# davawen/Simple-Raytracer

Measured on AMD Instinct MI355X. Metric: Mray/s at 1920x1080x1024spp, higher is better.
Workload: dtype f32; 1 GPU; BASELINE configs[1]: 7-shape sphere scene 1920x1080 1024spp; width=1920, height=1080, spp=1024, bounces=10, triangles=12, partition=single GPU, gather=none, mode=parity (fp-contract off, IEEE div/sqrt; canvas bit-identical to the CPU oracle)

## Files before the change

### simple-raytracer_amd/csrc/device_types.h

```cpp
#ifndef SRT_DEVICE_TYPES_H
#define SRT_DEVICE_TYPES_H

#include <stddef.h>
#include <stdint.h>

#include "../../include/srt_types.h"

struct ShapeRun {
	int32_t type;
	uint32_t first_shape;
	uint32_t count;
	uint32_t data_off;
};
struct BlockGroup {
	uint32_t code;
	uint32_t first[3];
};
static_assert(sizeof(BlockGroup) == 16, "BlockGroup 16 B");

struct WinnerRec {
	int32_t type;
	int32_t material;
	float vx, vy, vz, w;
	uint32_t first_wtri;
	float inv_w;
};
static_assert(sizeof(WinnerRec) == 32, "WinnerRec 32 B");

#define SRT_WTRI_FLOATS 9

typedef srt_bvh_node BvhNode;
#define SRT_BVH_FIRST_DWORD 11
#define SRT_BVH_TRI_FLOATS 9
#define SRT_BVH_LEAF_J 28
#define SRT_BVH_NONE 0xffffffffu
#define SRT_BVH_LEAF_BIT 0x80000000u
#define SRT_BVH_INDEX_MASK 0x0fffffffu
#define SRT_BVH_INDEX_MAX 0x01ffffffu
#define SRT_BVH_KEY_INF 0x7f800000u
#define SRT_BVH_TAG_MASK 31u
#define SRT_BVH_TAG_LEAF 16u
#define SRT_BVH_TAG(ref, slot) ((((ref) >> 31) << 4) | ((((ref) >> 28) & 3u) << 2) | (slot))
#define SRT_BVH_STACK_CAP 64
#ifndef SRT_BVH_LEAF_MAX
#define SRT_BVH_LEAF_MAX 3
#endif

#define SRT_REGION_MAX 56
#ifdef SRT_REGION_COUNT
#define SRT_WAVE_CTR_STRIDE (16 + 2 * SRT_REGION_MAX)
#else
#define SRT_WAVE_CTR_STRIDE 16
#endif
#define SRT_WAVE_CTR_SLOTS 8192

enum { SRT_CTR_RAYS = 0, SRT_CTR_SKY, SRT_CTR_TRI, SRT_CTR_TRI_PASS_U, SRT_CTR_NAN, SRT_CTR_PATHS, SRT_CTR_QUEUE, SRT_CTR_WATCHDOG, SRT_CTR_QUEUE2, SRT_CTR_COUNT };

#define SRT_MF_NO_SPECULAR 1
#define SRT_MF_PLAIN_COLORS 2

#define SRT_BLK_CODE(type, count) ((uint32_t)((type) + 1) | ((uint32_t)(count) << 2))
#define SRT_GROUP_CODE(b0, b1, b2) ((b0) | ((b1) << 8) | ((b2) << 16))
#define SRT_GC_PPS SRT_GROUP_CODE(SRT_BLK_CODE(SRT_SHAPE_PLANE, 2), SRT_BLK_CODE(SRT_SHAPE_PLANE, 1), SRT_BLK_CODE(SRT_SHAPE_SPHERE, 4))
#define SRT_GC_SSS SRT_GROUP_CODE(SRT_BLK_CODE(SRT_SHAPE_SPHERE, 4), SRT_BLK_CODE(SRT_SHAPE_SPHERE, 4), SRT_BLK_CODE(SRT_SHAPE_SPHERE, 4))
#define SRT_GC_PPP SRT_GROUP_CODE(SRT_BLK_CODE(SRT_SHAPE_PLANE, 2), SRT_BLK_CODE(SRT_SHAPE_PLANE, 2), SRT_BLK_CODE(SRT_SHAPE_PLANE, 2))
#define SRT_SCENE_CLASS_LIST(X) \
	X(1, SRT_GC_PPS, true)      \
	X(2, SRT_GC_PPS, false)     \
	X(3, SRT_GC_SSS, true)      \
	X(4, SRT_GC_PPP, true)
#define SRT_SCENE_CLASS_GENERAL 0

static inline size_t srt_scene_lds_bytes(size_t num_shapes, size_t num_materials, int num_models, size_t num_runs) {
	size_t scene = num_shapes * sizeof(WinnerRec) + num_materials * sizeof(srt_material);
	if (num_models == 0) scene += num_runs * (sizeof(BlockGroup) + 192);
	return scene <= 4608 ? scene : 0;
}

struct TraceParams {
	srt_render_data rd;
	srt_scene_data sd;
	const BlockGroup *runs;
	const float *run_data;
	const WinnerRec *winners;
	int32_t num_runs;
	int32_t num_materials;
	uint32_t lds_bytes;
	int32_t scene_class;
	const srt_shape *shapes;
	const srt_triangle *triangles;
	const srt_material *materials;
	const float *wtris;
	const float *sky;
	float *canvas;
	float *radiance;
	unsigned long long *counters;
	unsigned long long *wave_counters;
	unsigned long long *queue;
	unsigned long long total_items;
	uint32_t batch_samples;
	uint32_t first_sample;
	uint32_t job_items;
	uint32_t stage_off;
	int32_t sky_w, sky_h;
	float f_width, f_height, f_sky_w, f_sky_h;
	int32_t sun_focus_int;
	int32_t material_flags;
	int32_t num_models;
	int32_t rank, world, rows_per_block, owned_rows;
	int32_t use_bvh;
	const float *bvh_blocks;
	float *scan_queue;
	float inv_f_width, inv_f_height;
	uint32_t width_magic, width_shift;
	uint32_t rpb_magic, rpb_shift;
	uint32_t nbs_magic16;
	uint32_t pool_blocks;
	int32_t unit_materials;
	int32_t all_materials_ok;
};

static inline void srt_magic_u31(uint32_t d, uint32_t *magic, uint32_t *shift) {
	uint32_t l = 0;
	while (l < 32 && ((uint64_t)1 << l) < d) l++;
// ... 125 lines not shown
```

### simple-raytracer_amd/csrc/kernels.hip

```cpp
#include <hip/hip_runtime.h>

#include "detmath.h"
#include "device_types.h"
#include "tonemap.h"

#ifndef SRT_TEXTURED
#define SRT_TEXTURED 0
#endif
#if SRT_TEXTURED
#define SRT_TRACE_PARAMS TexTraceParams
#define SRT_FEATURE_PARAMS TexFeatureParams
#define srt_trace_kernel srt_trace_tex_kernel
#define srt_features_kernel srt_features_tex_kernel
#define srt_features_ids_kernel srt_features_ids_tex_kernel
#define srt_launch_trace srt_launch_trace_tex
#define srt_trace_resident_waves_per_cu srt_trace_tex_resident_waves_per_cu
#define srt_launch_features srt_launch_features_tex
#define srt_launch_features_ids srt_launch_features_ids_tex
int srt_trace_lds_floats(int has_models, int use_bvh);
#else
#define SRT_TRACE_PARAMS TraceParams
#define SRT_FEATURE_PARAMS FeatureParams
#endif

// ... 311 lines not shown
		tmin = t_key;
		best = idx;
	}
}

template <int N>
__device__ __forceinline__ void test_spheres(const Blk16 &s, f3 org, f3 dir, int idx0, float &tmin, int &best) {
	float bq[4], disc[4];
	bool slow = is_neg_zero(tmin);
#pragma unroll
	for (int i = 0; i < N; i++) {
		f3 L = mk(s.v[4 * i] - org.x, s.v[4 * i + 1] - org.y, s.v[4 * i + 2] - org.z);
		bq[i] = dot3(L, dir);
		float c = dot3(L, L) - s.v[4 * i + 3];
		disc[i] = bq[i] * bq[i] - c;
		slow = slow || dm_fabs(disc[i]) < 0x1p-96f;
	}
	if (__builtin_expect(any64(slow), 0)) {
#pragma unroll
		for (int i = 0; i < N; i++) {
			const float sq = __builtin_sqrtf(disc[i]);
			float t = bq[i] - sq;
			if (t < 0.0f) t = bq[i] + sq;
			if (!(disc[i] < 0.0f) && !(t < 0.0f) && t < tmin) tmin = t, best = idx0 + i;
		}
	} else {
		float dd[N], sq[N];
#pragma unroll
		for (int i = 0; i < N; i++) dd[i] = disc[i];
		sqrt_rsq_n<N, false>(dd, sq);
#pragma unroll
		for (int i = 0; i < N; i++) {
			const uint32_t k = min(dm_f2u(bq[i] - sq[i]), dm_f2u(bq[i] + sq[i]));
			take_if_closer(dm_u2f(k), idx0 + i, tmin, best);
		}
	}
}

__device__ __forceinline__ void test_planes2(const Blk16 &b, uint32_t count, f3 org, f3 dir, int idx0, float &tmin, int &best) {
#pragma unroll
	for (int i = 0; i < 2; i++) {
		if (i == 1 && count < 2u) break;
		f3 n = mk(b.v[8 * i + 4], b.v[8 * i + 5], b.v[8 * i + 6]);
		float denom = dot3(n, dir);
		float t = dot3(n, mk(b.v[8 * i] - org.x, b.v[8 * i + 1] - org.y, b.v[8 * i + 2] - org.z)) / denom;
		bool hit = !(t < 0.0f);
		if (hit && t < tmin) {
			tmin = t;
			best = idx0 + i;
		}
	}
}

__device__ __forceinline__ bool test_aabb(float lx, float ly, float lz, float hx, float hy, float hz, f3 org, f3 inv, float tmax) {
	float t0 = 0.0f, t1 = tmax;
	float a1 = (lx - org.x) * inv.x, a2 = (hx - org.x) * inv.x;
	t0 = dm_max(t0, dm_min(a1, a2));
	t1 = dm_min(t1, dm_max(a1, a2));
	a1 = (ly - org.y) * inv.y, a2 = (hy - org.y) * inv.y;
	t0 = dm_max(t0, dm_min(a1, a2));
	t1 = dm_min(t1, dm_max(a1, a2));
	a1 = (lz - org.z) * inv.z, a2 = (hz - org.z) * inv.z;
	t0 = dm_max(t0, dm_min(a1, a2));
	t1 = dm_min(t1, dm_max(a1, a2));
	return t0 < t1;
}

template <bool COUNT_TRIS>
__device__ __forceinline__ bool moller_trumbore(float v0x, float v0y, float v0z, float e1x, float e1y, float e1z, float e2x, float e2y,
                                                float e2z, f3 org, f3 dir, bool counted, float &t, uint32_t &n_tri_u SRT_RC_PARAM) {
	f3 e1 = mk(e1x, e1y, e1z), e2 = mk(e2x, e2y, e2z);
	f3 h = cross3(dir, e2);
	float a = dot3(e1, h);
	f3 sv = mk(org.x - v0x, org.y - v0y, org.z - v0z);
	float sh = dot3(sv, h);
	float aa = dm_fabs(a), ash = dm_fabs(sh);
	bool reject = (a == 0.0f) || (ash > aa * 1.001f) || ((sh * a < 0.0f) && (ash >= aa * 0.001f));
	bool ok = false;
	if (!reject) {
		SRT_REGION(EXTEND_TRI_EXACT);
		f3 q = cross3(sv, e1);
		float dv = dot3(dir, q);
		bool reject2 = false;
		if (!COUNT_TRIS) reject2 = ((dv * a < 0.0f) && (dm_fabs(dv) >= aa * 0.001f)) || (dm_fabs(sh + dv) > aa * 1.01f);
		if (!reject2) {
			SRT_REGION(EXTEND_TRI_DIV);
			float f = 1.0f / a;
			float u = f * sh;
			ok = !(u < 0.0f || u > 1.0f);
			if (COUNT_TRIS) n_tri_u += (ok && counted) ? 1u : 0u;
			float v = f * dv;
			ok = ok && !(v < 0.0f || u + v > 1.0f);
			t = f * dot3(e2, q);
			ok = ok && t > 0.0f;
		}
	}
	return ok;
}

template <bool COUNT_TRIS>
__device__ __forceinline__ void test_triangle(float v0x, float v0y, float v0z, float e1x, float e1y, float e1z, float e2x, float e2y,
                                              float e2z, f3 org, f3 dir, int idx, uint32_t j, uint32_t count, float &tmin, int &best,
                                              uint32_t &best_tri, uint32_t &n_tri_u SRT_RC_PARAM) {
	float t = 0.0f;
	if (moller_trumbore<COUNT_TRIS>(v0x, v0y, v0z, e1x, e1y, e1z, e2x, e2y, e2z, org, dir, j < count, t, n_tri_u SRT_RC_ARG) && t < tmin) {
		tmin = t;
// ... 371 lines not shown
__device__ __forceinline__ uint32_t popc64(unsigned long long m) { return (uint32_t)__builtin_popcountll(m); }
__device__ __forceinline__ uint32_t lane_rank(unsigned long long m) {
	return __builtin_amdgcn_mbcnt_hi((uint32_t)(m >> 32), __builtin_amdgcn_mbcnt_lo((uint32_t)m, 0u));
}
__device__ __forceinline__ unsigned long long lanes_below(uint32_t n) { return n >= 64u ? ~0ull : ((1ull << n) - 1ull); }

__device__ __forceinline__ void resolve_ring(const TraceParams &p, const float *__restrict__ ring, uint32_t n, int lane SRT_RC_PARAM) {
	asm volatile("s_waitcnt lgkmcnt(0)" ::: "memory");
	if ((uint32_t)lane < n) {
		SRT_REGION(SKY_RESOLVE);
		constexpr uint32_t RC = SRT_RING_CAP;
		const f3 d = mk(ring[0 * RC + lane], ring[1 * RC + lane], ring[2 * RC + lane]);
		f3 m = mk(ring[3 * RC + lane], ring[4 * RC + lane], ring[5 * RC + lane]);
		f3 c = mk(ring[6 * RC + lane], ring[7 * RC + lane], ring[8 * RC + lane]);
		const uint32_t item = dm_f2u(ring[9 * RC + lane]);
		m = m * sky_box(p, d);
		c = c + m;
		store_radiance(p.radiance, item, c);
	}
	asm volatile("" ::: "memory");
}
}

#ifndef SRT_TRACE_WAVES_PER_SIMD
#define SRT_TRACE_WAVES_PER_SIMD 5
#endif
#ifndef SRT_TRACE_WAVES_PER_SIMD_MODELS
#define SRT_TRACE_WAVES_PER_SIMD_MODELS 5
#endif
#ifndef SRT_TRACE_WAVES_PER_SIMD_BVH
#define SRT_TRACE_WAVES_PER_SIMD_BVH 5
#endif

constexpr uint32_t hq_fields(bool has_models) { return has_models ? 17u : 16u; }

struct GeneralScene {
	static constexpr bool FAST = false, NO_SPEC = false;
	static constexpr uint32_t CODE = 0;
};
template <uint32_t CODE_, bool NO_SPEC_>
struct OneGroupScene {
	static constexpr bool FAST = true, NO_SPEC = NO_SPEC_;
	static constexpr uint32_t CODE = CODE_;
};
template <uint32_t K>
__device__ __forceinline__ void test_block_of_class(const Blk16 &b, int base, f3 org, f3 dir, float &tmin, int &best) {
	if constexpr ((K & 3u) == SRT_SHAPE_SPHERE + 1u) {
		if constexpr (((K >> 2) & 7u) <= 2u) test_spheres<2>(b, org, dir, base, tmin, best);
		else test_spheres<4>(b, org, dir, base, tmin, best);
	} else if constexpr ((K & 3u) == SRT_SHAPE_PLANE + 1u) {
		test_planes2(b, (K >> 2) & 7u, org, dir, base, tmin, best);
	}
}

template <bool COUNT_TRIS, bool USE_LDS, bool HAS_MODELS, bool USE_BVH>
__global__ __launch_bounds__(64, USE_BVH ? SRT_TRACE_WAVES_PER_SIMD_BVH : HAS_MODELS ? SRT_TRACE_WAVES_PER_SIMD_MODELS : SRT_TRACE_WAVES_PER_SIMD) void srt_trace_kernel(const SRT_TRACE_PARAMS p) {
	using SC = GeneralScene;
#include "trace_body.inc"
}

#if !SRT_TEXTURED && !SRT_DIAG_ON && !defined(SRT_DUMMY_KIND) && !defined(SRT_DEV_KNOBS) && SRT_RING_CAP == 64
#define SRT_SCENE_CLASSES 1
template <uint32_t CODE, bool NO_SPEC>
__global__ __launch_bounds__(64, 6) void srt_trace_scene_kernel(const TraceParams p) {
	constexpr bool COUNT_TRIS = false, USE_LDS = true, HAS_MODELS = false, USE_BVH = false;
	using SC = OneGroupScene<CODE, NO_SPEC>;
#include "trace_body.inc"
}
#else
#define SRT_SCENE_CLASSES 0
#endif

#if !SRT_TEXTURED
namespace {
__device__ __forceinline__ float add_lum2(float s2, float r, float g, float b) {
	const float l = lum(r, g, b);
	return s2 + l * l;
}
}
template <bool MOMENTS>
__global__ __launch_bounds__(256) void srt_reduce_kernel(const ReduceParams p) {
	const uint32_t q = blockIdx.x * blockDim.x + threadIdx.x;
	if (q == 0u && p.queue_reset) *p.queue_reset = 0ull;
	if (q >= p.num_pixels) return;
	f3 c = mk(0.f, 0.f, 0.f);
	float s2 = 0.f;
	float4 *run = reinterpret_cast<float4 *>(p.running) + q;
	if (!p.first_batch) {
		float4 v = *run;
		c = mk(v.x, v.y, v.z);
		if (MOMENTS) s2 = v.w;
	}
	const uint32_t n = p.batch_samples;
	const float *__restrict__ r = p.radiance + (size_t)q * n * 3u;
	uint32_t k = 0;
	if ((n & 3u) == 0u) {
		const float4 *__restrict__ r4 = reinterpret_cast<const float4 *>(r);
#ifndef SRT_REDUCE_DEPTH
#define SRT_REDUCE_DEPTH 4
#endif
		for (; k + 4 * SRT_REDUCE_DEPTH <= n; k += 4 * SRT_REDUCE_DEPTH) {
			float4 v[3 * SRT_REDUCE_DEPTH];
#pragma unroll
			for (int i = 0; i < 3 * SRT_REDUCE_DEPTH; i++) v[i] = r4[i];
			r4 += 3 * SRT_REDUCE_DEPTH;
#pragma unroll
// ... 255 lines not shown
	for (int k = 0; k < 4; k++) {
		out_new[lane * 4u + k] = ra[k], out_ref[lane * 4u + k] = rb[k];
		bad += ra[k] != rb[k] ? 1u : 0u;
	}
	if (bad) atomicAdd(mismatches, bad);
}

void srt_launch_selftest_rare(int what, const uint32_t *in, uint32_t waves, uint32_t *out_new, uint32_t *out_ref, unsigned long long *mismatches, void *stream) {
	if (waves == 0) return;
	hipLaunchKernelGGL(srt_selftest_rare_kernel, dim3(waves), dim3(64), 0, (hipStream_t)stream, what, in, out_new, out_ref, mismatches);
}

int srt_trace_waves_per_simd(int has_models, int use_bvh) {
	return !has_models ? SRT_TRACE_WAVES_PER_SIMD : use_bvh ? SRT_TRACE_WAVES_PER_SIMD_BVH : SRT_TRACE_WAVES_PER_SIMD_MODELS;
}
int srt_scan_suspend_min(void) { return SRT_SCAN_SUSPEND_MIN; }
int srt_sub_job_items(int has_models, int use_bvh) { return !has_models ? SRT_SUB_PLAIN : use_bvh ? SRT_SUB_BVH : SRT_SUB_MODELS; }

int srt_trace_lds_floats(int has_models, int use_bvh) {
	int n = 10 * SRT_RING_CAP + (int)hq_fields(has_models) * (has_models ? (use_bvh ? SRT_HQ_CAP_BVH : SRT_HQ_CAP_MODELS) : SRT_HQ_CAP);
#ifdef SRT_REGION_COUNT
	n += 2 * SRT_REGION_MAX;
#endif
	return n;
}
#endif

namespace {
typedef void (*TraceKernel)(const SRT_TRACE_PARAMS);
TraceKernel pick_trace_kernel(bool models, bool use_bvh, bool use_lds, bool count_triangles) {
	if (!models) return use_lds ? srt_trace_kernel<false, true, false, false> : srt_trace_kernel<false, false, false, false>;
	if (use_bvh) {
		if (use_lds) return count_triangles ? srt_trace_kernel<true, true, true, true> : srt_trace_kernel<false, true, true, true>;
		return count_triangles ? srt_trace_kernel<true, false, true, true> : srt_trace_kernel<false, false, true, true>;
	}
	if (use_lds) return count_triangles ? srt_trace_kernel<true, true, true, false> : srt_trace_kernel<false, true, true, false>;
	return count_triangles ? srt_trace_kernel<true, false, true, false> : srt_trace_kernel<false, false, true, false>;
}
size_t scene_lds_bytes(const TraceParams &p) {
	return srt_scene_lds_bytes((size_t)p.sd.num_shapes, (size_t)p.num_materials, p.num_models, (size_t)p.num_runs);
}
TraceKernel pick_trace_kernel(const SRT_TRACE_PARAMS &p, bool use_lds, bool count_triangles) {
#if SRT_SCENE_CLASSES
	switch (p.scene_class) {
#define SRT_SCENE_CLASS_CASE(number, code, no_spec) \
	case number: return srt_trace_scene_kernel<code, no_spec>;
		SRT_SCENE_CLASS_LIST(SRT_SCENE_CLASS_CASE)
#undef SRT_SCENE_CLASS_CASE
	default: break;
	}
#endif
	return pick_trace_kernel(p.num_models > 0, p.use_bvh != 0, use_lds, count_triangles);
}
}

#if !SRT_TEXTURED
int srt_trace_has_scene_classes() { return SRT_SCENE_CLASSES; }
#endif

int srt_trace_resident_waves_per_cu(const SRT_TRACE_PARAMS &p, bool count_triangles) {
	const size_t scene_lds = scene_lds_bytes(p);
	const size_t need = scene_lds + (size_t)srt_trace_lds_floats(p.num_models > 0, p.use_bvh) * sizeof(float);
	int blocks = 0;
	if (hipOccupancyMaxActiveBlocksPerMultiprocessor(&blocks, pick_trace_kernel(p, scene_lds != 0, count_triangles), 64, need) != hipSuccess ||
	    blocks <= 0) {
		(void)hipGetLastError();
		blocks = 4 * srt_trace_waves_per_simd(p.num_models > 0, p.use_bvh);
	}
	return blocks;
}

void srt_launch_trace(SRT_TRACE_PARAMS p, bool count_triangles, int num_waves, void *stream) {
	if (p.total_items == 0 || num_waves <= 0) return;
	dim3 grid((unsigned)num_waves), block(64);
	const size_t scene_lds = scene_lds_bytes(p);
	p.lds_bytes = (uint32_t)scene_lds;
	p.stage_off = (uint32_t)(scene_lds / sizeof(float4));
	const size_t need = scene_lds + (size_t)srt_trace_lds_floats(p.num_models > 0, p.use_bvh) * sizeof(float);
	hipLaunchKernelGGL(pick_trace_kernel(p, scene_lds != 0, count_triangles), grid, block, need, (hipStream_t)stream, p);
}

#if !SRT_TEXTURED
void srt_launch_reduce(const ReduceParams &p, void *stream) {
	if (p.num_pixels == 0) return;
	hipLaunchKernelGGL(srt_reduce_kernel<false>, dim3((p.num_pixels + 255) / 256), dim3(256), 0, (hipStream_t)stream, p);
}

void srt_launch_prepass(const PrepassParams &p, uint64_t max_tris_per_model, void *stream) {
	if (p.num_shapes <= 0 || max_tris_per_model == 0) return;
	unsigned gx = (unsigned)((max_tris_per_model + 255) / 256);
	if (gx > 4096) gx = 4096;
	dim3 grid(gx, (unsigned)p.num_shapes), block(256);
	hipLaunchKernelGGL(srt_prepass_kernel, grid, block, 0, (hipStream_t)stream, p);
}

void srt_launch_resolve(const ResolveParams &p, void *stream) {
	if (p.num_pixels == 0) return;
	unsigned gx = (p.num_pixels + 255) / 256;
	if (gx > 4096) gx = 4096;
	hipLaunchKernelGGL(srt_resolve_kernel, dim3(gx), dim3(256), 0, (hipStream_t)stream, p);
}

void srt_launch_reduce_moments(const ReduceParams &p, void *stream) {
	if (p.num_pixels == 0) return;
	hipLaunchKernelGGL(srt_reduce_kernel<true>, dim3((p.num_pixels + 255) / 256), dim3(256), 0, (hipStream_t)stream, p);
}

#endif

void srt_launch_features(const SRT_FEATURE_PARAMS &p, void *stream) {
	if (p.num_pixels == 0 || p.feature_samples == 0) return;
	typedef void (*FeatureKernel)(const SRT_FEATURE_PARAMS);
	const bool models = p.tp.num_models > 0, bvh = p.tp.use_bvh != 0;
	const FeatureKernel k = !models ? srt_features_kernel<false, false> : bvh ? srt_features_kernel<true, true> : srt_features_kernel<true, false>;
	hipLaunchKernelGGL(k, dim3((p.num_pixels + 63u) / 64u), dim3(64), 0, (hipStream_t)stream, p);
}

void srt_launch_features_ids(const SRT_FEATURE_PARAMS &p, uint32_t *shape_ids, void *stream) {
	if (p.num_pixels == 0 || p.feature_samples == 0) return;
	typedef void (*FeatureKernel)(const SRT_FEATURE_PARAMS, uint32_t *);
	const bool models = p.tp.num_models > 0, bvh = p.tp.use_bvh != 0;
	const FeatureKernel k = !models ? srt_features_ids_kernel<false, false> : bvh ? srt_features_ids_kernel<true, true> : srt_features_ids_kernel<true, false>;
	hipLaunchKernelGGL(k, dim3((p.num_pixels + 63u) / 64u), dim3(64), 0, (hipStream_t)stream, p, shape_ids);
}
```

### simple-raytracer_amd/csrc/trace_body.inc

```
	extern __shared__ float4 lds[];
	constexpr bool FAST = SC::FAST;
	static_assert(!FAST || (USE_LDS && !HAS_MODELS && !USE_BVH && !COUNT_TRIS), "scene classes exist for sphere / plane scenes staged in LDS");
	constexpr uint32_t FK0 = SC::CODE & 255u, FK1 = (SC::CODE >> 8) & 255u, FK2 = (SC::CODE >> 16) & 255u;
	constexpr int FN0 = (int)((FK0 >> 2) & 7u), FN1 = (int)((FK1 >> 2) & 7u), FN2 = (int)((FK2 >> 2) & 7u), FN = FN0 + FN1 + FN2;
	constexpr uint32_t SUB = USE_BVH ? SRT_SUB_BVH : HAS_MODELS ? SRT_SUB_MODELS : SRT_SUB_PLAIN;
	const int width = p.rd.width;
	const int lane = threadIdx.x;
	const int ns = p.rd.num_samples;
	const int nb = p.rd.num_bounces;
	const int n_shapes = FAST ? FN : p.sd.num_shapes;
	const bool all_materials_ok = FAST || p.all_materials_ok != 0;
	const bool unit_materials = FAST || p.unit_materials != 0;
	const bool no_specular = FAST ? SC::NO_SPEC : (p.material_flags & (SRT_MF_NO_SPECULAR | SRT_MF_PLAIN_COLORS)) == (SRT_MF_NO_SPECULAR | SRT_MF_PLAIN_COLORS);
	const BlockGroup *__restrict__ runs = p.runs;
	const float *__restrict__ run_data = p.run_data;
	const float *__restrict__ wtris = p.wtris;

	if (FAST) {
		const float4 *__restrict__ gw = reinterpret_cast<const float4 *>(p.winners);
		const float4 *__restrict__ gm = reinterpret_cast<const float4 *>(p.materials);
		const float4 *__restrict__ gd4 = reinterpret_cast<const float4 *>(p.run_data);
		static_assert(2 * FN <= 64, "one pass stages the winner records");
		if (lane < 2 * FN) lds[lane] = gw[lane];
		if (lane < 12) lds[2 * FN + lane] = gd4[lane];
		for (int i = threadIdx.x; i < 4 * p.num_materials; i += 64) lds[2 * FN + 12 + i] = gm[i];
		__syncthreads();
	} else if (USE_LDS) {
		const float4 *__restrict__ gw = reinterpret_cast<const float4 *>(p.winners);
		const float4 *__restrict__ gm = reinterpret_cast<const float4 *>(p.materials);
		for (int i = threadIdx.x; i < 2 * n_shapes; i += 64) lds[i] = gw[i];
		for (int i = threadIdx.x; i < 4 * p.num_materials; i += 64) lds[2 * n_shapes + i] = gm[i];
		if (!HAS_MODELS) {
			const float4 *__restrict__ gh4 = reinterpret_cast<const float4 *>(p.runs);
			const float4 *__restrict__ gd4 = reinterpret_cast<const float4 *>(p.run_data);
			float4 *__restrict__ dst = lds + 2 * n_shapes + 4 * p.num_materials;
			for (int i = threadIdx.x; i < p.num_runs; i += 64) dst[i] = gh4[i];
			for (int i = threadIdx.x; i < 12 * p.num_runs; i += 64) dst[p.num_runs + i] = gd4[i];
		}
		__syncthreads();
	}
	uint32_t gh_code = 0;
	int gh_f0 = 0, gh_f1 = 0, gh_f2 = 0;
	if (!FAST && USE_LDS && !HAS_MODELS && p.num_runs > 0) {
		const float4 hv = lds[2 * n_shapes + 4 * p.num_materials];
		gh_code = (uint32_t)__builtin_amdgcn_readfirstlane((int)f2u(hv.x));
		gh_f0 = __builtin_amdgcn_readfirstlane((int)f2u(hv.y)), gh_f1 = __builtin_amdgcn_readfirstlane((int)f2u(hv.z));
		gh_f2 = __builtin_amdgcn_readfirstlane((int)f2u(hv.w));
	}

	const uint32_t total_items = (uint32_t)p.total_items;
	const uint32_t nbs = p.batch_samples;
	const unsigned long long own_chunks_end = (unsigned long long)gridDim.x * p.job_items;
	uint32_t chunk_cur = 0, chunk_end = 0;
	if ((unsigned long long)blockIdx.x * p.job_items < (unsigned long long)total_items) {
		chunk_cur = blockIdx.x * p.job_items;
		chunk_end = (total_items - chunk_cur < p.job_items) ? total_items : chunk_cur + p.job_items;
	}
	bool queue_dry = (total_items == 0);
	uint32_t sj_next = 0, sj_end = 0, sj_off = 0, sj_qpix = 0;
	float *__restrict__ ring = reinterpret_cast<float *>(lds + p.stage_off);
	float *__restrict__ hq = ring + 10u * (uint32_t)SRT_RING_CAP;
	constexpr uint32_t HQ = USE_BVH ? SRT_HQ_CAP_BVH : HAS_MODELS ? SRT_HQ_CAP_MODELS : SRT_HQ_CAP;
#ifdef SRT_REGION_COUNT
	uint32_t *region_ctr = reinterpret_cast<uint32_t *>(hq + hq_fields(HAS_MODELS) * HQ);
	for (int i = lane; i < 2 * SRT_REGION_MAX; i += 64) region_ctr[i] = 0u;
	__syncthreads();
#endif
	constexpr bool SUSPEND = HAS_MODELS && !USE_BVH;
	constexpr uint32_t SQ = (uint32_t)SRT_SQ_CAP, PK = (uint32_t)SRT_PK_CAP;
	float *__restrict__ sq_base = SUSPEND ? const_cast<float *>((const float *)SRT_COLD(p).scan_queue) + (size_t)SRT_POOL_CTL_WORDS + (SRT_COLD(p).pool_blocks != 0u ? SRT_POOL_REC_FLOATS : (size_t)0) + (size_t)blockIdx.x * (size_t)SRT_SCAN_QUEUE_FLOATS : nullptr;
	float *__restrict__ pk = sq_base + 2u * 20u * SQ;
	uint32_t sq_count0 = 0, sq_count1 = 0, pk_count = 0;
	const bool use_pool = SUSPEND && SRT_COLD(p).pool_blocks != 0u;
	bool pool_leave = false, pool_last = false;
	uint32_t w_pool_taken = 0, w_pool_given = 0, w_pool_last_taken = 0;
	uint32_t ring_count = 0, hq_head = 0, hq_count = 0;

	f3 org = mk(0.f, 0.f, 0.f), dir = mk(0.f, 0.f, 0.f), mask = mk(1.f, 1.f, 1.f), color = mk(0.f, 0.f, 0.f);
	uint32_t seed = 0;
	uint32_t item = 0;
	int bounce = 0;
	int best = -1;
	uint32_t best_tri = 0;
	BvhStackEntry bvh_stack[USE_BVH ? SRT_BVH_STACK_CAP + 1 : 1];
	const float4 *__restrict__ bvh_blocks = reinterpret_cast<const float4 *>(p.bvh_blocks);
	unsigned long long actm = 0ull;
	unsigned long long resm = 0ull;
	float tmin = DM_INF_F;
	uint32_t pos = 0;
	unsigned long long w_rays = 0;
	uint32_t w_sky = 0, w_paths = 0, w_iter = 0, w_shade = 0;
	uint32_t w_scans = 0, w_scan_lanes = 0;
	uint32_t n_tri = 0, n_tri_u = 0;
	uint32_t idle_spins = 0;
	constexpr uint32_t SHADE_THR = ((uint32_t)SRT_SHADE_MIN - 1u) < HQ ? ((uint32_t)SRT_SHADE_MIN - 1u) : HQ;
	uint32_t shade_thr = queue_dry ? 0u : SHADE_THR;

	SRT_CLK_DECL;
	SRT_REGION(PROLOGUE);
	for (;;) {
		SRT_REGION(LOOP_HEAD);
		unsigned long long hitm = 0ull, missm = 0ull, finm = 0ull;
		uint32_t susp = 0u;
		int key = -1;
		if (SRT_DIAG_ON) w_iter++;
		SRT_CLK(6);
#ifdef SRT_DUMMY_KIND
#include "issue_probe.h"
#endif
		if (actm != 0ull) {
			constexpr bool MASKED = HAS_MODELS;
			if (!FAST && nb <= 0) {
				finm = actm;
			} else {
				w_rays += SUSPEND ? popc64(actm & ~resm) : popc64(actm);
// ... 45 lines not shown
										SRT_REGION(EXTEND_SUSPEND);
										float *__restrict__ sq = sq_base + sid * (20u * SQ);
										const uint32_t e = held + __builtin_amdgcn_mbcnt_hi((uint32_t)(want >> 32), __builtin_amdgcn_mbcnt_lo((uint32_t)want, 0u));
										sq[0 * SQ + e] = org.x, sq[1 * SQ + e] = org.y, sq[2 * SQ + e] = org.z;
										sq[3 * SQ + e] = dir.x, sq[4 * SQ + e] = dir.y, sq[5 * SQ + e] = dir.z;
										sq[6 * SQ + e] = mask.x, sq[7 * SQ + e] = mask.y, sq[8 * SQ + e] = mask.z;
										sq[9 * SQ + e] = color.x, sq[10 * SQ + e] = color.y, sq[11 * SQ + e] = color.z;
										sq[12 * SQ + e] = dm_u2f(seed), sq[13 * SQ + e] = dm_u2f((uint32_t)bounce), sq[14 * SQ + e] = dm_u2f(item);
										sq[15 * SQ + e] = tmin, sq[16 * SQ + e] = dm_u2f((uint32_t)best), sq[17 * SQ + e] = dm_u2f(best_tri);
										sq[18 * SQ + e] = dm_u2f(bidx);
										part = false;
										susp = 1u + sid;
									}
									if (sid) sq_pushed1 += n_want;
									else sq_pushed0 += n_want;
									scan0 = false;
								}
							}
							if (SUSPEND && !COUNT_TRIS && ((code >> 5) & 1u)) {
								const unsigned long long sb = ballot64(scan0);
								if (scan0) {
									w_scan_lanes++;
									if ((sb & ((1ull << lane) - 1ull)) == 0ull) w_scans++;
								}
							}
							if (scan0) {
								if (USE_BVH) {
									walk_bvh<COUNT_TRIS>(bvh_blocks, bvh_stack, f2u(b.v[3]), org, dir, base, tmin, best, best_tri, n_tri, n_tri_u SRT_RC_ARG);
								} else {
									if (COUNT_TRIS) n_tri += f2u(b.v[7]);
									test_triangles<COUNT_TRIS>(wtris, f2u(b.v[3]), f2u(b.v[7]), org, dir, base, tmin, best, best_tri, n_tri_u SRT_RC_ARG);
								}
							}
							if (((code >> 2) & 7u) > 1u && on && test_aabb(b.v[8], b.v[9], b.v[10], b.v[12], b.v[13], b.v[14], org, inv, tmin)) {
								if (USE_BVH) {
									walk_bvh<COUNT_TRIS>(bvh_blocks, bvh_stack, f2u(b.v[11]), org, dir, base + 1, tmin, best, best_tri, n_tri, n_tri_u SRT_RC_ARG);
								} else {
									if (COUNT_TRIS) n_tri += f2u(b.v[15]);
									test_triangles<COUNT_TRIS>(wtris, f2u(b.v[11]), f2u(b.v[15]), org, dir, base + 1, tmin, best, best_tri, n_tri_u SRT_RC_ARG);
								}
							}
						}
					};
					const int n_groups = FAST ? 0 : p.num_runs;
					if (FAST) {
						const float4 *__restrict__ lb = lds + 2 * FN;
						auto ld_lds = [&](int k) {
							Blk16 b;
							const float4 q0 = lb[4 * k], q1 = lb[4 * k + 1], q2 = lb[4 * k + 2], q3 = lb[4 * k + 3];
							b.v[0] = q0.x, b.v[1] = q0.y, b.v[2] = q0.z, b.v[3] = q0.w, b.v[4] = q1.x, b.v[5] = q1.y, b.v[6] = q1.z, b.v[7] = q1.w;
							b.v[8] = q2.x, b.v[9] = q2.y, b.v[10] = q2.z, b.v[11] = q2.w, b.v[12] = q3.x, b.v[13] = q3.y, b.v[14] = q3.z, b.v[15] = q3.w;
							return b;
						};
						test_block_of_class<FK0>(ld_lds(0), 0, org, dir, tmin, best);
						if (FK1 != 0u) test_block_of_class<FK1>(ld_lds(1), FN0, org, dir, tmin, best);
						if (FK2 != 0u) test_block_of_class<FK2>(ld_lds(2), FN0 + FN1, org, dir, tmin, best);
					}
					for (int g = 0; g < n_groups; g++) {
						SRT_REGION(EXTEND_GROUP);
						float gh[4];
						ld_uniform<4, 16>(reinterpret_cast<const float *>(runs + g), gh);
						const uint32_t code = f2u(gh[0]);
						const float *__restrict__ gd = run_data + 48 * g;
						if (!HAS_MODELS && USE_LDS) {
							const float4 *__restrict__ lgh = lds + 2 * n_shapes + 4 * p.num_materials;
							const float4 *__restrict__ lb = lgh + n_groups + 12 * g;
							const uint32_t lcode = gh_code;
							const int f0 = gh_f0, f1 = gh_f1, f2 = gh_f2;
							auto ld_lds = [&](int k) {
								Blk16 b;
								const float4 q0 = lb[4 * k], q1 = lb[4 * k + 1], q2 = lb[4 * k + 2], q3 = lb[4 * k + 3];
								b.v[0] = q0.x, b.v[1] = q0.y, b.v[2] = q0.z, b.v[3] = q0.w, b.v[4] = q1.x, b.v[5] = q1.y, b.v[6] = q1.z, b.v[7] = q1.w;
								b.v[8] = q2.x, b.v[9] = q2.y, b.v[10] = q2.z, b.v[11] = q2.w, b.v[12] = q3.x, b.v[13] = q3.y, b.v[14] = q3.z, b.v[15] = q3.w;
								return b;
							};
							test_block(ld_lds(0), lcode & 255u, f0, 0u, 0);
							if ((lcode >> 8) & 255u) test_block(ld_lds(1), (lcode >> 8) & 255u, f1, 0u, 1);
							if ((lcode >> 16) & 255u) test_block(ld_lds(2), (lcode >> 16) & 255u, f2, 0u, 2);
							int ng = n_groups;
							asm volatile("" : "+s"(ng));
							if (ng > 1) {
								const float4 hv = lgh[g + 1 < n_groups ? g + 1 : 0];
								gh_code = (uint32_t)__builtin_amdgcn_readfirstlane((int)f2u(hv.x));
								gh_f0 = __builtin_amdgcn_readfirstlane((int)f2u(hv.y)), gh_f1 = __builtin_amdgcn_readfirstlane((int)f2u(hv.z));
								gh_f2 = __builtin_amdgcn_readfirstlane((int)f2u(hv.w));
							}
						} else if (!HAS_MODELS) {
							const Blk16 b0 = ld_blk16(gd), b1 = ld_blk16(gd + 16), b2 = ld_blk16(gd + 32);
							test_block(b0, code & 255u, (int)f2u(gh[1]), 0u, 0);
							test_block(b1, (code >> 8) & 255u, (int)f2u(gh[2]), 0u, 1);
							test_block(b2, (code >> 16) & 255u, (int)f2u(gh[3]), 0u, 2);
						} else {
							test_block(ld_blk16(gd), code & 255u, (int)f2u(gh[1]), 3u * g, 0);
							if ((code >> 8) & 255u) test_block(ld_blk16(gd + 16), (code >> 8) & 255u, (int)f2u(gh[2]), 3u * g + 1u, 1);
							if ((code >> 16) & 255u) test_block(ld_blk16(gd + 32), (code >> 16) & 255u, (int)f2u(gh[3]), 3u * g + 2u, 2);
						}
					}
					SRT_REGION(EXTEND_FINISH);
						if (!SUSPEND || part) {
							key = best;
							if (!all_materials_ok) {
								key = -1;
								if (best >= 0) key = USE_LDS ? (int)f2u(reinterpret_cast<const float *>(lds)[8 * best + 1]) : p.winners[best].material;
							}
							if (!MASKED) org = org + dir * tmin;
							else if (key >= 0) org = org + dir * tmin;
						}
					}
				}
// ... 366 lines not shown
					const uint32_t e = pk_count + lane_rank(actm);
					if (in_mask(actm)) {
						pk[0 * PK + e] = org.x, pk[1 * PK + e] = org.y, pk[2 * PK + e] = org.z;
						pk[3 * PK + e] = dir.x, pk[4 * PK + e] = dir.y, pk[5 * PK + e] = dir.z;
						pk[6 * PK + e] = mask.x, pk[7 * PK + e] = mask.y, pk[8 * PK + e] = mask.z;
						pk[9 * PK + e] = color.x, pk[10 * PK + e] = color.y, pk[11 * PK + e] = color.z;
						pk[12 * PK + e] = dm_u2f(seed), pk[13 * PK + e] = dm_u2f((uint32_t)bounce), pk[14 * PK + e] = dm_u2f(item);
					}
					pk_count += n_act;
				}
				const uint32_t sid = full0 ? 0u : full1 ? 1u : (sq_count1 > sq_count0 ? 1u : 0u);
				const uint32_t held = sid ? sq_count1 : sq_count0;
				const uint32_t n_pop = held < 64u ? held : 64u;
				const float *__restrict__ sq = sq_base + sid * (20u * SQ);
				asm volatile("s_waitcnt vmcnt(0)" ::: "memory");
				actm = lanes_below(n_pop);
				if (in_mask(actm)) {
					const uint32_t e = held - 1u - (uint32_t)lane;
					org = mk(ld(sq + 0 * SQ + e), ld(sq + 1 * SQ + e), ld(sq + 2 * SQ + e));
					dir = mk(ld(sq + 3 * SQ + e), ld(sq + 4 * SQ + e), ld(sq + 5 * SQ + e));
					mask = mk(ld(sq + 6 * SQ + e), ld(sq + 7 * SQ + e), ld(sq + 8 * SQ + e));
					color = mk(ld(sq + 9 * SQ + e), ld(sq + 10 * SQ + e), ld(sq + 11 * SQ + e));
					seed = dm_f2u(ld(sq + 12 * SQ + e)), bounce = (int)dm_f2u(ld(sq + 13 * SQ + e)), item = dm_f2u(ld(sq + 14 * SQ + e));
					tmin = ld(sq + 15 * SQ + e), best = (int)dm_f2u(ld(sq + 16 * SQ + e)), best_tri = dm_f2u(ld(sq + 17 * SQ + e));
					pos = dm_f2u(ld(sq + 18 * SQ + e));
				}
				asm volatile("" ::: "memory");
				resm = actm;
				if (sid) sq_count1 -= n_pop;
				else sq_count0 -= n_pop;
				n_act = n_pop;
			} else if (pk_count != 0u && n_act != 64u) {
				SRT_REGION(REFILL_UNPARK);
				asm volatile("s_waitcnt vmcnt(0)" ::: "memory");
				const uint32_t n_pop = 64u - n_act < pk_count ? 64u - n_act : pk_count;
				const unsigned long long fm = ~actm;
				const uint32_t rank = lane_rank(fm);
				const unsigned long long um = ballot64(rank < n_pop) & fm;
				if (in_mask(um)) {
					const uint32_t e = pk_count - 1u - rank;
					org = mk(ld(pk + 0 * PK + e), ld(pk + 1 * PK + e), ld(pk + 2 * PK + e));
					dir = mk(ld(pk + 3 * PK + e), ld(pk + 4 * PK + e), ld(pk + 5 * PK + e));
					mask = mk(ld(pk + 6 * PK + e), ld(pk + 7 * PK + e), ld(pk + 8 * PK + e));
					color = mk(ld(pk + 9 * PK + e), ld(pk + 10 * PK + e), ld(pk + 11 * PK + e));
					seed = dm_f2u(ld(pk + 12 * PK + e)), bounce = (int)dm_f2u(ld(pk + 13 * PK + e)), item = dm_f2u(ld(pk + 14 * PK + e));
				}
				asm volatile("" ::: "memory");
				pk_count -= n_pop;
				actm |= um;
				n_act += n_pop;
			}
		}
		const uint32_t n_free = 64u - n_act;
		if (!queue_dry && n_free >= (uint32_t)SRT_REFILL_MIN && (!SUSPEND || pk_count == 0u)) {
			const unsigned long long freem = ~actm;
			const uint32_t rank = lane_rank(freem);
			uint32_t given = 0;
			uint32_t off = 0, qpix = 0;
			while (given < n_free) {
				SRT_REGION(REFILL_LOOP);
				if (sj_next == sj_end) {
					SRT_REGION(REFILL_OPEN);
					if (chunk_cur == chunk_end) {
						SRT_REGION(REFILL_CURSOR);
						unsigned long long start = total_items;
						if (own_chunks_end < (unsigned long long)total_items) {
							if (lane == 0) start = atomicAdd((unsigned long long *)SRT_COLD(p).queue, (unsigned long long)SRT_COLD(p).job_items);
							const uint32_t lo = (uint32_t)__builtin_amdgcn_readfirstlane((int)(uint32_t)start);
							const uint32_t hi = (uint32_t)__builtin_amdgcn_readfirstlane((int)(uint32_t)(start >> 32));
							start = (((unsigned long long)hi << 32) | lo) + own_chunks_end;
						}
						if (start >= (unsigned long long)total_items) {
							queue_dry = true;
							shade_thr = 0u;
							break;
						}
						chunk_cur = (uint32_t)start;
						const uint32_t job_items = SRT_COLD(p).job_items;
						chunk_end = (total_items - chunk_cur < job_items) ? total_items : chunk_cur + job_items;
					}
					const uint32_t left = chunk_end - chunk_cur;
					const uint32_t n = left < SUB ? left : SUB;
					const uint32_t q0 = chunk_cur / nbs;
					sj_next = chunk_cur, sj_end = chunk_cur + n, sj_qpix = q0, sj_off = chunk_cur - q0 * nbs;
					chunk_cur += n;
					continue;
				}
				SRT_REGION(REFILL_TAKE);
				const uint32_t avail = sj_end - sj_next;
				const uint32_t take = avail < n_free - given ? avail : n_free - given;
				const uint32_t r = rank - given;
				const unsigned long long takem = ballot64(r < take) & freem;
				if (in_mask(takem)) {
					item = sj_next + r;
					off = sj_off + r;
					qpix = sj_qpix;
				}
				sj_next += take, sj_off += take;
				given += take;
				w_paths += take;
			}
			const unsigned long long gotm = ballot64(rank < given) & freem;
			actm |= gotm;
			if (in_mask(gotm)) {
				SRT_REGION(CAMERA);
				const auto &c = SRT_COLD(p);
				static_assert(SUB <= 128u, "off / nbs by the 16-bit reciprocal is exact for off < 256 and nbs < 128 only (tests/csrc/magic_check.cpp)");
				const uint32_t dq = (nbs >= SUB) ? (off >= nbs ? 1u : 0u) : (off * c.nbs_magic16) >> 16;
				const uint32_t q = qpix + dq;
				const uint32_t sample = c.first_sample + (off - dq * nbs);
				const uint32_t lrow = (__umulhi(q, c.width_magic) + q) >> c.width_shift;
				const int px = (int)(q - lrow * (uint32_t)width);
				int py = (int)lrow;
				if (c.world != 1) {
					const uint32_t lb = (__umulhi(lrow, c.rpb_magic) + lrow) >> c.rpb_shift;
					py = (int)((lb * (uint32_t)c.world + (uint32_t)c.rank) * (uint32_t)c.rows_per_block + (lrow - lb * (uint32_t)c.rows_per_block));
				}
				const uint32_t id = (uint32_t)px + (uint32_t)py * (uint32_t)width;
				seed = (sample + id * (uint32_t)ns) * c.rd.time * 5304u;
				float ndc_x = div_by_rcp((float)px + random_float(seed), c.f_width, c.inv_f_width);
				float ndc_y = div_by_rcp((float)py + random_float(seed), c.f_height, c.inv_f_height);
				float sx = ((2.f * ndc_x - 1.f) * c.rd.aspect_ratio) * c.rd.fov_scale;
				float sy = (1.f - 2.f * ndc_y) * c.rd.fov_scale;
				const f3 c0 = mk(c.rd.camera_to_world[0].x, c.rd.camera_to_world[0].y, c.rd.camera_to_world[0].z);
				const f3 c1 = mk(c.rd.camera_to_world[1].x, c.rd.camera_to_world[1].y, c.rd.camera_to_world[1].z);
				const f3 c2 = mk(c.rd.camera_to_world[2].x, c.rd.camera_to_world[2].y, c.rd.camera_to_world[2].z);
				org = mk(c.rd.camera_to_world[3].x, c.rd.camera_to_world[3].y, c.rd.camera_to_world[3].z);
				dir = normalize3(mat_cols_by_vec(c0, c1, c2, org, mk(sx, sy, -1.0f), 0.0f));
				mask = mk(1.f, 1.f, 1.f);
				color = mk(0.f, 0.f, 0.f);
				bounce = 0;
			}
		}

		SRT_CLK(5);
		SRT_REGION(LOOP_TAIL);
		if (queue_dry) {
			if (actm == 0ull && hq_count == 0u && (sq_count0 | sq_count1 | pk_count) == 0u) {
				if (!use_pool || pool_leave || pool_last) break;
				if (++idle_spins > (1u << 20)) {
					if (lane == 0) atomicAdd((unsigned long long *)SRT_COLD(p).counters + SRT_CTR_WATCHDOG, 1ull);
					break;
				}
			} else {
				idle_spins = 0;
			}
		}
	}
	SRT_REGION(EPILOGUE);
	if (ring_count != 0u) resolve_ring(p, ring, ring_count, lane SRT_RC_ARG);

	unsigned long long t3 = COUNT_TRIS ? n_tri : w_scans, t4 = COUNT_TRIS ? n_tri_u : w_scan_lanes;
	if (COUNT_TRIS || SUSPEND) {
		for (int off = 32; off > 0; off >>= 1) {
			t3 += __shfl_down(t3, off);
			t4 += __shfl_down(t4, off);
		}
	}
	if (lane == 0) {
		unsigned long long *__restrict__ w = (unsigned long long *)SRT_COLD(p).wave_counters + (size_t)blockIdx.x * SRT_WAVE_CTR_STRIDE;
		w[0] += w_rays;
		w[1] += w_sky;
		w[2] += w_paths;
		if (COUNT_TRIS) {
			w[3] += t3;
			w[4] += t4;
		} else if (SUSPEND) {
			w[8] += t3;
			w[9] += t4;
#ifndef SRT_PHASE_CLOCK
			w[10] += w_pool_taken, w[11] += w_pool_given, w[12] += (unsigned long long)w_pool_taken * w_pool_taken, w[13] += w_pool_last_taken;
#endif
		}
		w[6] += w_iter;
		w[7] += w_shade;
#ifdef SRT_PHASE_CLOCK
		for (int i = 0; i < 7; i++) w[8 + i] += clk_t[i];
		w[15] += __builtin_amdgcn_s_memtime() - clk_start;
#endif
	}
#ifdef SRT_REGION_COUNT
	__syncthreads();
	{
		unsigned long long *__restrict__ w = (unsigned long long *)SRT_COLD(p).wave_counters + (size_t)blockIdx.x * SRT_WAVE_CTR_STRIDE + 16;
		for (int i = lane; i < 2 * SRT_REGION_MAX; i += 64) w[i] += region_ctr[i];
	}
#endif
```

### simple-raytracer_amd/tracer.py

```python
import ctypes as C
from pathlib import Path

import numpy as np

from . import build as B
from . import records as R

PKG = Path(__file__).resolve().parent
import os

LIB_PATH = Path(os.environ["SRT_LIB"]) if os.environ.get("SRT_LIB") else PKG / "lib" / "libsrt_hip.so"

ABI_SYMBOLS = [
    "srt_create", "srt_destroy", "srt_last_error", "srt_set_skybox", "srt_update_scene", "srt_clear_canvas",
    "srt_render", "srt_render_async", "srt_trace", "srt_set_radiance_budget", "srt_resolve", "srt_resolve_external", "srt_synchronize", "srt_read_canvas", "srt_read_argb",
    "srt_get_counters", "srt_set_count_triangles", "srt_reset_counters", "srt_last_kernel_ms", "srt_set_kernel_timers", "srt_last_trace_kernel_ms", "srt_last_trace_launches",
    "srt_device_buffers", "srt_bind_canvas", "srt_bind_stream", "srt_set_partition",
    "srt_partition_owned_rows", "srt_partition_padded_rows", "srt_partition_global_row",
    "srt_partition_unpermute", "srt_selftest_math", "srt_selftest_rare_lanes", "srt_version", "srt_set_acceleration", "srt_acceleration_info", "srt_bvh_build_host", "srt_bvh_wide_host", "srt_debug_counters", "srt_debug_region_counters",
    "srt_comm_unique_id", "srt_comm_init", "srt_gather", "srt_resolve_gathered", "srt_gathered_buffers", "srt_read_gathered",
    "srt_group_create", "srt_group_destroy", "srt_group_last_error", "srt_group_size", "srt_group_tracer", "srt_group_set_skybox",
    "srt_group_set_acceleration", "srt_group_update_scene", "srt_group_clear_canvas", "srt_group_trace_and_gather", "srt_group_render",
    "srt_group_read_canvas", "srt_group_get_counters", "srt_render_pipelined", "srt_pipeline_flush", "srt_unpermute_device",
    "srt_denoise_defaults", "srt_set_denoise", "srt_resolve_denoised", "srt_read_denoised", "srt_read_denoise_inputs",
# ... 531 lines not shown

    def clear_canvas(self):
        self._check(self.lib.srt_clear_canvas(self._h))

    def render(self, ticks_stopped, output=None):
        if output is None:
            output = np.zeros(self.owned_rows * self.width * 4, np.uint8)
        assert output.dtype == np.uint8 and output.size >= self.owned_rows * self.width * 4
        rd = R.as_records(self.options, R.RENDER_DATA)
        self._check(self.lib.srt_render(self._h, _ptr(rd), ticks_stopped, _ptr(output)))
        return output

    def render_async(self, ticks_stopped, output):
        assert output.dtype == np.uint8 and output.size >= self.owned_rows * self.width * 4
        rd = R.as_records(self.options, R.RENDER_DATA)
        self._check(self.lib.srt_render_async(self._h, _ptr(rd), ticks_stopped, _ptr(output)))

    def trace(self):
        rd = R.as_records(self.options, R.RENDER_DATA)
        self._check(self.lib.srt_trace(self._h, _ptr(rd)))

    def set_radiance_budget(self, nbytes):
        self._check(self.lib.srt_set_radiance_budget(self._h, nbytes))

    def resolve(self, ticks_stopped):
        self._check(self.lib.srt_resolve(self._h, ticks_stopped))

    def resolve_external(self, canvas_ptr, num_pixels, ticks_stopped, argb_ptr):
        self._check(self.lib.srt_resolve_external(self._h, C.c_void_p(canvas_ptr), num_pixels, ticks_stopped, C.c_void_p(argb_ptr)))

    def synchronize(self):
        self._check(self.lib.srt_synchronize(self._h))

    def read_canvas(self):
        out = np.zeros((self.owned_rows, self.width, 4), np.float32)
        self._check(self.lib.srt_read_canvas(self._h, _ptr(out)))
        return out

    def read_argb(self):
        out = np.zeros((self.owned_rows, self.width, 4), np.uint8)
        self._check(self.lib.srt_read_argb(self._h, _ptr(out)))
        return out

    def counters(self):
        c = Counters()
        self._check(self.lib.srt_get_counters(self._h, C.byref(c)))
        return c.as_dict()

    def debug_counters(self):
        out = (C.c_uint64 * 18)()
        self.lib.srt_debug_counters.argtypes = [C.c_void_p, C.POINTER(C.c_uint64)]
        self._check(self.lib.srt_debug_counters(self._h, out))
        v = [int(x) for x in out]
        return {"rays": v[0], "sky": v[1], "paths": v[2], "orphans": v[5] & ((1 << 40) - 1), "evictions": v[5] >> 40,
                "iterations": v[6], "shade_phases": v[7], "waves_per_cu": v[8], "grid": v[9],
                "phase_cycles": dict(zip(("extend", "ring", "shade", "park", "deliver", "refill", "head", "kernel"), v[10:18])),
                "scans": v[10], "scan_lanes": v[11],
                "pool_taken": v[12], "pool_given": v[13], "pool_taken_sq": v[14], "pool_last_taken": v[15]}

    def debug_region_counters(self):
        out = (C.c_uint64 * 128)()
        n = C.c_int(0)
        self.lib.srt_debug_region_counters.argtypes = [C.c_void_p, C.POINTER(C.c_uint64), C.c_int, C.POINTER(C.c_int)]
        self._check(self.lib.srt_debug_region_counters(self._h, out, 128, C.byref(n)))
        return [(int(out[2 * i]), int(out[2 * i + 1])) for i in range(n.value // 2)]

    def reset_counters(self):
        self._check(self.lib.srt_reset_counters(self._h))

    def count_triangles(self, enable=True):
        self._check(self.lib.srt_set_count_triangles(self._h, 1 if enable else 0))

    def set_acceleration(self, mode):
        self._check(self.lib.srt_set_acceleration(self._h, int(mode)))

    def acceleration_info(self):
        out = (C.c_uint64 * 7)()
        self._check(self.lib.srt_acceleration_info(self._h, out))
        return dict(zip(("nodes", "leaves", "depth", "build_us", "models_built", "models_reused", "models_refitted"), (int(v) for v in out)))

    def set_acceleration_refit(self, mode):
        self._check(self.lib.srt_set_acceleration_refit(self._h, int(mode)))

    def acceleration_refit_info(self):
        out = (C.c_uint64 * 4)()
        self._check(self.lib.srt_acceleration_refit_info(self._h, out))
        return dict(zip(("models", "inner_blocks", "launches"), (int(v) for v in out)))

    def last_refit_kernel_ms(self):
        a = C.c_float()
        self._check(self.lib.srt_last_refit_kernel_ms(self._h, C.byref(a)))
        return a.value

    def read_bvh_blocks(self):
        n = C.c_size_t(0)
        self._check(self.lib.srt_read_bvh_blocks(self._h, None, 0, C.byref(n)))
        blocks = np.zeros((n.value, 32), np.uint32)
        self._check(self.lib.srt_read_bvh_blocks(self._h, _ptr(blocks), len(blocks), C.byref(n)))
        return blocks

    def selftest_math(self, stride=1):
        out = (C.c_uint64 * 16)()
        self._check(self.lib.srt_selftest_math(self._h, stride, out))
        return [int(v) for v in out]

    def selftest_rare_lanes(self, what, words):
        words = np.ascontiguousarray(words, np.uint32)
# ... 219 lines not shown
```

Baseline: 89650 Mray/s.

## Precompute camera-origin sphere/plane records for primary-ray intersection in LDS

Adds a camera phase in which all active lanes are primary rays sharing the camera origin. For that phase, sphere tests use precomputed L=center-org and c=|L|^2-r^2, and plane tests use a precomputed numerator, all stored in extra LDS. This removes per-ray subtraction and dot work on primary rays. In exchange it adds LDS use that can lower occupancy, per-iteration phase bookkeeping, and a counter that repurposes the orphan/eviction debug slot. It also risks bit-parity with the CPU oracle because the arithmetic is reordered.

```diff
diff --git a/simple-raytracer_amd/csrc/device_types.h b/simple-raytracer_amd/csrc/device_types.h
--- a/simple-raytracer_amd/csrc/device_types.h
+++ b/simple-raytracer_amd/csrc/device_types.h
@@ -70,6 +70,11 @@
 	X(3, SRT_GC_SSS, true)      \
 	X(4, SRT_GC_PPP, true)
 #define SRT_SCENE_CLASS_GENERAL 0
+static constexpr inline uint32_t srt_class_cam_records(uint32_t code) {
+	return ((code & 3u) == SRT_SHAPE_SPHERE + 1u ? 4u : 0u) + (((code >> 8) & 3u) == SRT_SHAPE_SPHERE + 1u ? 4u : 0u) +
+	       (((code >> 16) & 3u) == SRT_SHAPE_SPHERE + 1u ? 4u : 0u);
+}
+static constexpr inline size_t srt_class_cam_lds_bytes(uint32_t code) { return 16u * (size_t)srt_class_cam_records(code); }
 
 static inline size_t srt_scene_lds_bytes(size_t num_shapes, size_t num_materials, int num_models, size_t num_runs) {
 	size_t scene = num_shapes * sizeof(WinnerRec) + num_materials * sizeof(srt_material);
diff --git a/simple-raytracer_amd/csrc/kernels.hip b/simple-raytracer_amd/csrc/kernels.hip
--- a/simple-raytracer_amd/csrc/kernels.hip
+++ b/simple-raytracer_amd/csrc/kernels.hip
@@ -387,6 +387,85 @@
 	}
 }
 
+#ifndef SRT_CAM_FORM
+#define SRT_CAM_FORM 1
+#endif
+#ifndef SRT_CAM_SPHERE_VOTE
+#define SRT_CAM_SPHERE_VOTE 1
+#endif
+template <int N>
+__device__ __forceinline__ void test_spheres_cam(const float4 *__restrict__ cam, f3 dir, unsigned long long actm, int idx0, float &tmin, int &best) {
+	float bq[4], disc[4];
+	bool slow = is_neg_zero(tmin);
+#pragma unroll
+	for (int i = 0; i < N; i++) {
+		const float4 lc = cam[i];
+		bq[i] = dot3(mk(lc.x, lc.y, lc.z), dir);
+		disc[i] = bq[i] * bq[i] - lc.w;
+		slow = slow || dm_fabs(disc[i]) < 0x1p-96f;
+	}
+	if (__builtin_expect(any64(slow), 0)) {
+#pragma unroll
+		for (int i = 0; i < N; i++) {
+			const float sq = __builtin_sqrtf(disc[i]);
+			float t = bq[i] - sq;
+			if (t < 0.0f) t = bq[i] + sq;
+			if (!(disc[i] < 0.0f) && !(t < 0.0f) && t < tmin) tmin = t, best = idx0 + i;
+		}
+	} else {
+#if SRT_CAM_SPHERE_VOTE
+#pragma unroll
+		for (int i = 0; i < N; i++) {
+			if ((ballot64(disc[i] >= 0.0f) & actm) != 0ull) {
+				const float sq = sqrt_rsq(disc[i]);
+				const uint32_t k = min(dm_f2u(bq[i] - sq), dm_f2u(bq[i] + sq));
+				take_if_closer(dm_u2f(k), idx0 + i, tmin, best);
+			}
+		}
+#else
+		float dd[N], sq[N];
+#pragma unroll
+		for (int i = 0; i < N; i++) dd[i] = disc[i];
+		sqrt_rsq_n<N, false>(dd, sq);
+#pragma unroll
+		for (int i = 0; i < N; i++) {
+			const uint32_t k = min(dm_f2u(bq[i] - sq[i]), dm_f2u(bq[i] + sq[i]));
+			take_if_closer(dm_u2f(k), idx0 + i, tmin, best);
+		}
+#endif
+	}
+}
+__device__ __forceinline__ void test_planes2_cam(const float4 *__restrict__ blk, uint32_t count, f3 dir, int idx0, float &tmin, int &best) {
+#pragma unroll
+	for (int i = 0; i < 2; i++) {
+		if (i == 1 && count < 2u) break;
+		const float4 nq = blk[2 * i + 1];
+		const float num = reinterpret_cast<const float *>(blk + 2 * i)[3];
+		const float denom = dot3(mk(nq.x, nq.y, nq.z), dir);
+		const float t = num / denom;
+		const bool hit = !(t < 0.0f);
+		if (hit && t < tmin) {
+			tmin = t;
+			best = idx0 + i;
+		}
+	}
+}
+template <uint32_t K>
+__device__ __forceinline__ void cam_records_of_block(float4 *__restrict__ blk, float4 *__restrict__ cam, f3 org, int lane) {
+	if constexpr ((K & 3u) == SRT_SHAPE_SPHERE + 1u) {
+		if (lane < 4) {
+			const float4 s = blk[lane];
+			const f3 L = mk(s.x - org.x, s.y - org.y, s.z - org.z);
+			const float c = dot3(L, L) - s.w;
+			cam[lane] = make_float4(L.x, L.y, L.z, c);
+		}
+	} else if constexpr ((K & 3u) == SRT_SHAPE_PLANE + 1u) {
+		if (lane < 2) {
+			const float4 pq = blk[2 * lane], nq = blk[2 * lane + 1];
+			reinterpret_cast<float *>(blk + 2 * lane)[3] = dot3(mk(nq.x, nq.y, nq.z), mk(pq.x - org.x, pq.y - org.y, pq.z - org.z));
+		}
+	}
+}
 __device__ __forceinline__ bool test_aabb(float lx, float ly, float lz, float hx, float hy, float hz, f3 org, f3 inv, float tmax) {
 	float t0 = 0.0f, t1 = tmax;
 	float a1 = (lx - org.x) * inv.x, a2 = (hx - org.x) * inv.x;
@@ -864,6 +943,15 @@
 		test_planes2(b, (K >> 2) & 7u, org, dir, base, tmin, best);
 	}
 }
+template <uint32_t K>
+__device__ __forceinline__ void test_block_of_class_cam(const float4 *__restrict__ blk, const float4 *__restrict__ cam, int base, f3 dir, unsigned long long actm, float &tmin, int &best) {
+	if constexpr ((K & 3u) == SRT_SHAPE_SPHERE + 1u) {
+		if constexpr (((K >> 2) & 7u) <= 2u) test_spheres_cam<2>(cam, dir, actm, base, tmin, best);
+		else test_spheres_cam<4>(cam, dir, actm, base, tmin, best);
+	} else if constexpr ((K & 3u) == SRT_SHAPE_PLANE + 1u) {
+		test_planes2_cam(blk, (K >> 2) & 7u, dir, base, tmin, best);
+	}
+}
 
 template <bool COUNT_TRIS, bool USE_LDS, bool HAS_MODELS, bool USE_BVH>
 __global__ __launch_bounds__(64, USE_BVH ? SRT_TRACE_WAVES_PER_SIMD_BVH : HAS_MODELS ? SRT_TRACE_WAVES_PER_SIMD_MODELS : SRT_TRACE_WAVES_PER_SIMD) void srt_trace_kernel(const SRT_TRACE_PARAMS p) {
@@ -1225,6 +1313,19 @@
 #endif
 	return pick_trace_kernel(p.num_models > 0, p.use_bvh != 0, use_lds, count_triangles);
 }
+size_t trace_lds_bytes(const SRT_TRACE_PARAMS &p, size_t scene_lds) {
+	size_t need = scene_lds + (size_t)srt_trace_lds_floats(p.num_models > 0, p.use_bvh) * sizeof(float);
+#if SRT_SCENE_CLASSES
+	switch (p.scene_class) {
+#define SRT_SCENE_CLASS_CASE(number, code, no_spec) \
+	case number: need += srt_class_cam_lds_bytes(code); break;
+		SRT_SCENE_CLASS_LIST(SRT_SCENE_CLASS_CASE)
+#undef SRT_SCENE_CLASS_CASE
+	default: break;
+	}
+#endif
+	return need;
+}
 }
 
 #if !SRT_TEXTURED
@@ -1233,7 +1334,7 @@
 
 int srt_trace_resident_waves_per_cu(const SRT_TRACE_PARAMS &p, bool count_triangles) {
 	const size_t scene_lds = scene_lds_bytes(p);
-	const size_t need = scene_lds + (size_t)srt_trace_lds_floats(p.num_models > 0, p.use_bvh) * sizeof(float);
+	const size_t need = trace_lds_bytes(p, scene_lds);
 	int blocks = 0;
 	if (hipOccupancyMaxActiveBlocksPerMultiprocessor(&blocks, pick_trace_kernel(p, scene_lds != 0, count_triangles), 64, need) != hipSuccess ||
 	    blocks <= 0) {
@@ -1249,7 +1350,7 @@
 	const size_t scene_lds = scene_lds_bytes(p);
 	p.lds_bytes = (uint32_t)scene_lds;
 	p.stage_off = (uint32_t)(scene_lds / sizeof(float4));
-	const size_t need = scene_lds + (size_t)srt_trace_lds_floats(p.num_models > 0, p.use_bvh) * sizeof(float);
+	const size_t need = trace_lds_bytes(p, scene_lds);
 	hipLaunchKernelGGL(pick_trace_kernel(p, scene_lds != 0, count_triangles), grid, block, need, (hipStream_t)stream, p);
 }
 
diff --git a/simple-raytracer_amd/csrc/trace_body.inc b/simple-raytracer_amd/csrc/trace_body.inc
--- a/simple-raytracer_amd/csrc/trace_body.inc
+++ b/simple-raytracer_amd/csrc/trace_body.inc
@@ -61,6 +61,19 @@
 	float *__restrict__ ring = reinterpret_cast<float *>(lds + p.stage_off);
 	float *__restrict__ hq = ring + 10u * (uint32_t)SRT_RING_CAP;
 	constexpr uint32_t HQ = USE_BVH ? SRT_HQ_CAP_BVH : HAS_MODELS ? SRT_HQ_CAP_MODELS : SRT_HQ_CAP;
+	constexpr bool CAM = FAST && SRT_CAM_FORM != 0;
+	constexpr uint32_t CS1 = srt_class_cam_records(FK0), CS2 = srt_class_cam_records(FK0 | (FK1 << 8));
+	float4 *__restrict__ cam_rec = reinterpret_cast<float4 *>(hq + hq_fields(HAS_MODELS) * HQ);
+	if (CAM) {
+		const auto &c = SRT_COLD(p);
+		const f3 cam_org = mk(c.rd.camera_to_world[3].x, c.rd.camera_to_world[3].y, c.rd.camera_to_world[3].z);
+		cam_records_of_block<FK0>(lds + 2 * FN, cam_rec, cam_org, lane);
+		cam_records_of_block<FK1>(lds + 2 * FN + 4, cam_rec + CS1, cam_org, lane);
+		cam_records_of_block<FK2>(lds + 2 * FN + 8, cam_rec + CS2, cam_org, lane);
+		__syncthreads();
+	}
+	bool cam_phase = false;
+	unsigned long long w_cam = 0;
 #ifdef SRT_REGION_COUNT
 	uint32_t *region_ctr = reinterpret_cast<uint32_t *>(hq + hq_fields(HAS_MODELS) * HQ);
 	for (int i = lane; i < 2 * SRT_REGION_MAX; i += 64) region_ctr[i] = 0u;
@@ -212,9 +225,16 @@
 							b.v[8] = q2.x, b.v[9] = q2.y, b.v[10] = q2.z, b.v[11] = q2.w, b.v[12] = q3.x, b.v[13] = q3.y, b.v[14] = q3.z, b.v[15] = q3.w;
 							return b;
 						};
-						test_block_of_class<FK0>(ld_lds(0), 0, org, dir, tmin, best);
-						if (FK1 != 0u) test_block_of_class<FK1>(ld_lds(1), FN0, org, dir, tmin, best);
-						if (FK2 != 0u) test_block_of_class<FK2>(ld_lds(2), FN0 + FN1, org, dir, tmin, best);
+						if (CAM && cam_phase) {
+							w_cam += (1ull << 36) + popc64(actm);
+							test_block_of_class_cam<FK0>(lb, cam_rec, 0, dir, actm, tmin, best);
+							if (FK1 != 0u) test_block_of_class_cam<FK1>(lb + 4, cam_rec + CS1, FN0, dir, actm, tmin, best);
+							if (FK2 != 0u) test_block_of_class_cam<FK2>(lb + 8, cam_rec + CS2, FN0 + FN1, dir, actm, tmin, best);
+						} else {
+							test_block_of_class<FK0>(ld_lds(0), 0, org, dir, tmin, best);
+							if (FK1 != 0u) test_block_of_class<FK1>(ld_lds(1), FN0, org, dir, tmin, best);
+							if (FK2 != 0u) test_block_of_class<FK2>(ld_lds(2), FN0 + FN1, org, dir, tmin, best);
+						}
 					}
 					for (int g = 0; g < n_groups; g++) {
 						SRT_REGION(EXTEND_GROUP);
@@ -687,6 +707,7 @@
 			}
 		}
 		const uint32_t n_free = 64u - n_act;
+		if (CAM) cam_phase = false;
 		if (!queue_dry && n_free >= (uint32_t)SRT_REFILL_MIN && (!SUSPEND || pk_count == 0u)) {
 			const unsigned long long freem = ~actm;
 			const uint32_t rank = lane_rank(freem);
@@ -737,6 +758,7 @@
 			}
 			const unsigned long long gotm = ballot64(rank < given) & freem;
 			actm |= gotm;
+			if (CAM) cam_phase = n_act == 0u;
 			if (in_mask(gotm)) {
 				SRT_REGION(CAMERA);
 				const auto &c = SRT_COLD(p);
@@ -807,6 +829,7 @@
 			w[10] += w_pool_taken, w[11] += w_pool_given, w[12] += (unsigned long long)w_pool_taken * w_pool_taken, w[13] += w_pool_last_taken;
 #endif
 		}
+		if (CAM) w[5] += w_cam;
 		w[6] += w_iter;
 		w[7] += w_shade;
 #ifdef SRT_PHASE_CLOCK
diff --git a/simple-raytracer_amd/tracer.py b/simple-raytracer_amd/tracer.py
--- a/simple-raytracer_amd/tracer.py
+++ b/simple-raytracer_amd/tracer.py
@@ -607,7 +607,8 @@
         self.lib.srt_debug_counters.argtypes = [C.c_void_p, C.POINTER(C.c_uint64)]
         self._check(self.lib.srt_debug_counters(self._h, out))
         v = [int(x) for x in out]
-        return {"rays": v[0], "sky": v[1], "paths": v[2], "orphans": v[5] & ((1 << 40) - 1), "evictions": v[5] >> 40,
+        return {"rays": v[0], "sky": v[1], "paths": v[2], "orphans": 0, "evictions": 0,
+                "camera_phases": v[5] >> 36, "camera_phase_rays": v[5] & ((1 << 36) - 1),
                 "iterations": v[6], "shade_phases": v[7], "waves_per_cu": v[8], "grid": v[9],
                 "phase_cycles": dict(zip(("extend", "ring", "shade", "park", "deliver", "refill", "head", "kernel"), v[10:18])),
                 "scans": v[10], "scan_lanes": v[11],
```

New measurement: 91680 Mray/s, median of 6. 1.02x the previous value.
